# cloudflare/sliceslice-rs

Hardware: AMD Instinct MI355X
Metric: haystack GB/s scanned (and % HBM roofline), 16-byte needle, 1/2/4/8 MI355X (higher is better)
Workload: dtype u8

## Files before the change

### sliceslice-rs_amd/csrc/scan_filters.hpp

```cpp
#pragma once
#include <hip/hip_runtime.h>
#include <stddef.h>
#include <stdint.h>

#include <type_traits>

namespace ss {

constexpr int kWave = 64;
constexpr int kBlock = 256;
constexpr int kWavesPerBlock = kBlock / kWave;
constexpr int kMaxBlock = 512;
constexpr int kMaxWavesPerBlock = kMaxBlock / kWave;
constexpr unsigned kPeekFromBlock = 1024;
#ifndef SS_BATCH_MIN_TILES
#define SS_BATCH_MIN_TILES 8
#endif
constexpr uint64_t kBatchMinTiles = SS_BATCH_MIN_TILES;
constexpr int kFindOffsetBits = 40;
constexpr int kNeedleLds = 2048;

typedef uint32_t u32x4 __attribute__((ext_vector_type(4)));

struct Problem {
// ... 81 lines not shown
__device__ __forceinline__ void fold_ascii_chunk(u32x4 &A)
{
    A.x = fold_ascii4(A.x); A.y = fold_ascii4(A.y); A.z = fold_ascii4(A.z); A.w = fold_ascii4(A.w);
}
__device__ __forceinline__ void fold_ascii_chunk_keep(u32x4 &A, uint32_t keepx4)
{
    A.x = fold_ascii4_keep(A.x, keepx4); A.y = fold_ascii4_keep(A.y, keepx4);
    A.z = fold_ascii4_keep(A.z, keepx4); A.w = fold_ascii4_keep(A.w, keepx4);
}
template <bool FOLD> __device__ __forceinline__ uint32_t hay_u32(uint32_t x, uint32_t keepx4) { return FOLD ? fold_ascii4_keep(x, keepx4) : x; }
template <bool FOLD> __device__ __forceinline__ uint8_t hay_u8(uint8_t b, uint32_t keepx4)
{
    return FOLD && (uint8_t)(b - 'A') < 26 && b != (uint8_t)keepx4 ? (uint8_t)(b | 0x20) : b;
}

struct __attribute__((packed, aligned(1))) UnalignedU32 {
    uint32_t v;
};

template <bool FOLD = false>
__device__ __forceinline__ bool verify_candidate(const uint8_t *hay, const uint8_t *needle, uint64_t n, const uint8_t *s_needle,
                                                 uint64_t i, uint32_t keepx4 = 0)
{
    const uint8_t *h = hay + i;
    const uint64_t n_lds = n < (uint64_t)kNeedleLds ? n : (uint64_t)kNeedleLds;
    uint64_t k = 0;
    for (; k + 16 <= n_lds; k += 16) {
        const uint32_t a0 = hay_u32<FOLD>(reinterpret_cast<const UnalignedU32 *>(h + k)->v, keepx4), a1 = hay_u32<FOLD>(reinterpret_cast<const UnalignedU32 *>(h + k + 4)->v, keepx4);
        const uint32_t a2 = hay_u32<FOLD>(reinterpret_cast<const UnalignedU32 *>(h + k + 8)->v, keepx4), a3 = hay_u32<FOLD>(reinterpret_cast<const UnalignedU32 *>(h + k + 12)->v, keepx4);
        const u32x4 nd = *reinterpret_cast<const u32x4 *>(s_needle + k);
        if (((a0 ^ nd.x) | (a1 ^ nd.y) | (a2 ^ nd.z) | (a3 ^ nd.w)) != 0) return false;
    }
    for (; k + 4 <= n_lds; k += 4)
        if (hay_u32<FOLD>(reinterpret_cast<const UnalignedU32 *>(h + k)->v, keepx4) != *reinterpret_cast<const uint32_t *>(s_needle + k))
            return false;
    for (; k < n_lds; ++k)
        if (hay_u8<FOLD>(h[k], keepx4) != s_needle[k]) return false;
    for (; k + 4 <= n; k += 4)
        if (hay_u32<FOLD>(reinterpret_cast<const UnalignedU32 *>(h + k)->v, keepx4) != reinterpret_cast<const UnalignedU32 *>(needle + k)->v)
            return false;
    for (; k < n; ++k)
        if (hay_u8<FOLD>(h[k], keepx4) != needle[k]) return false;
    return true;
}

template <bool FOLD = false>
__device__ __forceinline__ bool same_bytes(const uint8_t *hb, uint32_t off, const uint8_t *nd, uint32_t count, uint32_t keepx4 = 0)
{
    auto u32 = [](const uint8_t *p, uint32_t o) { return reinterpret_cast<const UnalignedU32 *>(p + o)->v; };
    auto group = [&](uint32_t at, uint32_t len) {
        const uint32_t o3 = at + len - 4;
        if (hay_u32<FOLD>(u32(hb, off + at), keepx4) != u32(nd, at)) return false;
        if (hay_u32<FOLD>(u32(hb, off + o3), keepx4) != u32(nd, o3)) return false;
        if (len <= 8) return true;
        const uint32_t o1 = at + 4, o2 = at + len - 8;
        if (hay_u32<FOLD>(u32(hb, off + o1), keepx4) != u32(nd, o1)) return false;
        return hay_u32<FOLD>(u32(hb, off + o2), keepx4) == u32(nd, o2);
    };
    if (count < 4) {
        if (count == 0) return true;
        const uint32_t mid = count >> 1, last = count - 1;
        return (uint32_t)((hay_u8<FOLD>(hb[off], keepx4) ^ nd[0]) | (hay_u8<FOLD>(hb[off + mid], keepx4) ^ nd[mid]) | (hay_u8<FOLD>(hb[off + last], keepx4) ^ nd[last])) == 0;
    }
    for (uint32_t k = 0; k + 16 < count; k += 16)
        if (!group(k, 16)) return false;
    const uint32_t base = count > 16 ? count - 16 : 0;
    return group(base, count - base);
}


__device__ __forceinline__ void position_diffs(const u32x4 &B, uint32_t nlx4, uint32_t w[4])
{
    w[0] = B.x ^ nlx4;
    w[1] = B.y ^ nlx4;
    w[2] = B.z ^ nlx4;
    w[3] = B.w ^ nlx4;
}

template <int Q, bool ONE_BYTE>
__device__ __forceinline__ void filter_piece(const u32x4 &A, const uint32_t w[4], const uint32_t wl[4],
                                             const Problem &pr, uint32_t g[4])
{
    const uint32_t d0 = A.x ^ pr.n0x4, d1 = A.y ^ pr.n0x4, d2 = A.z ^ pr.n0x4, d3 = A.w ^ pr.n0x4;
    if (ONE_BYTE) {
        g[0] = zero_byte_flags(d0); g[1] = zero_byte_flags(d1); g[2] = zero_byte_flags(d2); g[3] = zero_byte_flags(d3);
        return;
    }
    uint32_t x[8];
#pragma unroll
    for (int j = 0; j < 4; ++j) {
        x[j] = w[j];
        x[4 + j] = (j <= Q) ? from_next_lane_or(wl[j], w[j]) : 0u;
    }
    g[0] = zero_byte_flags(d0 | __builtin_amdgcn_alignbyte(x[Q + 1], x[Q + 0], pr.r));
    g[1] = zero_byte_flags(d1 | __builtin_amdgcn_alignbyte(x[Q + 2], x[Q + 1], pr.r));
    g[2] = zero_byte_flags(d2 | __builtin_amdgcn_alignbyte(x[Q + 3], x[Q + 2], pr.r));
    g[3] = zero_byte_flags(d3 | __builtin_amdgcn_alignbyte(x[Q + 4], x[Q + 3], pr.r));
}

template <int Q, int Q3>
__device__ __forceinline__ void filter_piece3(const u32x4 &A, const uint32_t NX[4], const Problem &pr, uint32_t g[4])
{
    constexpr int QM = Q > Q3 ? Q : Q3;
    uint32_t x[8];
    x[0] = A.x; x[1] = A.y; x[2] = A.z; x[3] = A.w;
    x[4] = from_next_lane_or(NX[0], A.x);
    x[5] = QM >= 1 ? from_next_lane_or(NX[1], A.y) : 0u;
    x[6] = QM >= 2 ? from_next_lane_or(NX[2], A.z) : 0u;
    x[7] = QM >= 3 ? from_next_lane_or(NX[3], A.w) : 0u;
    uint32_t y[5], z[5];
#pragma unroll
    for (int k = 0; k < 5; ++k) {
        y[k] = x[Q + k] ^ pr.nlx4;
        z[k] = x[Q3 + k] ^ pr.n3x4;
    }
#pragma unroll
    for (int j = 0; j < 4; ++j)
        g[j] = zero_byte_flags((x[j] ^ pr.n0x4) | __builtin_amdgcn_alignbyte(y[j + 1], y[j], pr.r) |
                               __builtin_amdgcn_alignbyte(z[j + 1], z[j], pr.r3));
}


__host__ __device__ constexpr inline int byte_rarity_rank(uint8_t b)
{
    if (b == ' ') return 255;
    if (b >= 'a' && b <= 'z') {
        const uint8_t kLetter[26] = { 242,  174,  206,  214,  250,  190,  186,
                                          222,  234,  162,  166,  210,  198,  230,
                                          238,  178,  154,  218,  226,  246,  202,
                                          170,  194,  158,  182,  150};
        return kLetter[b - 'a'];
    }
    if (b == 0) return 200;
    if (b == '\n' || b == '\r' || b == '\t') return 140;
    if (b >= '0' && b <= '9') return 120;
    if (b == '.' || b == ',' || b == '-' || b == '_' || b == '/' || b == ':' || b == '"' || b == '=') return 110;
    if (b >= 'A' && b <= 'Z') return 100;
    if (b >= 0x21 && b <= 0x7E) return 60;
    if (b == 0xFF) return 50;
    return 20;
}

constexpr int kRefineWindow = 32;
constexpr uint32_t kFarFirst = 10;
#ifndef SS_REFINE_BYTES_PER_BALLOT
#define SS_REFINE_BYTES_PER_BALLOT 1
#endif
#ifndef SS_EXACT_REFINE_STEPS
#define SS_EXACT_REFINE_STEPS 2
#endif
constexpr uint32_t kExactRefineSteps = SS_EXACT_REFINE_STEPS;
constexpr uint32_t kExactSparseLanes = 24;
constexpr uint32_t kRefineBytesPerBallot = SS_REFINE_BYTES_PER_BALLOT;

__host__ __device__ inline uint32_t build_refine_order(const uint8_t *needle, uint64_t n, uint64_t position,
                                                       uint64_t idx[2], uint64_t val[2], uint64_t position3 = ~0ull)
{
    uint8_t ks[2][kRefineWindow];
    int rk[2][kRefineWindow];
    uint32_t cnt[2] = {0, 0};
    const int lim = n < (uint64_t)kRefineWindow ? (int)n : kRefineWindow;
    for (int K = 1; K < lim; ++K) {
        if ((uint64_t)K == position || (uint64_t)K == position3) continue;
        const int g = K >= 16 ? 0 : 1;
        const int r = byte_rarity_rank(needle[K]);
        int at = (int)cnt[g];
        while (at > 0 && rk[g][at - 1] > r) {
            rk[g][at] = rk[g][at - 1];
            ks[g][at] = ks[g][at - 1];
            --at;
        }
        rk[g][at] = r;
        ks[g][at] = (uint8_t)K;
        ++cnt[g];
    }
    idx[0] = idx[1] = val[0] = val[1] = 0;
    uint32_t m = 0;
    auto emit = [&](uint8_t K) {
        idx[m >> 3] |= (uint64_t)K << (8 * (m & 7));
        val[m >> 3] |= (uint64_t)needle[K] << (8 * (m & 7));
        ++m;
    };
    uint32_t far_used = 0;
    for (; far_used < cnt[0] && far_used < kFarFirst; ++far_used) emit(ks[0][far_used]);
    for (uint32_t t = 0; t < cnt[1] && m < 15; ++t) emit(ks[1][t]);
    for (; far_used < cnt[0] && m < 15; ++far_used) emit(ks[0][far_used]);
    return m;
}

__device__ __forceinline__ uint32_t build_refine_order_wave(const uint8_t *needle, uint64_t n, uint64_t position,
                                                            int lane, uint64_t idx[2], uint64_t val[2], uint64_t position3 = ~0ull)
{
    const int lim = n < (uint64_t)kRefineWindow ? (int)n : kRefineWindow;
    const bool valid = lane >= 1 && lane < lim && (uint64_t)lane != position && (uint64_t)lane != position3;
    const uint32_t b = valid ? needle[lane] : 0u;
    const int r = byte_rarity_rank((uint8_t)b);
    const int cls = !valid ? -1 : (r < 64 ? 0 : (r < 128 ? 1 : (r < 192 ? 2 : 3)));
    uint64_t i0 = 0, i1 = 0, v0 = 0, v1 = 0;
    uint32_t m = 0;
    auto take = [&](uint32_t mask, uint32_t cap) {
        while (mask && m < cap) {
            const int K = __ffs((int)mask) - 1;
            mask &= mask - 1;
            const uint64_t v = (uint32_t)__builtin_amdgcn_readlane((int)b, K) & 0xFF;
            const uint32_t sh = 8 * (m & 7);
            if (m < 8) { i0 |= (uint64_t)K << sh; v0 |= v << sh; }
            else { i1 |= (uint64_t)K << sh; v1 |= v << sh; }
            ++m;
        }
    };
#pragma unroll 1
    for (int c = 0; c < 4; ++c) take((uint32_t)__ballot(cls == c) & 0xFFFF0000u, kFarFirst);
#pragma unroll 1
    for (int c = 0; c < 4; ++c) take((uint32_t)__ballot(cls == c) & 0x0000FFFFu, 15u);
    idx[0] = i0; idx[1] = i1; val[0] = v0; val[1] = v1;
    return m;
}

struct NextPiece {
    u32x4 N;
    int kind;
};

__device__ __forceinline__ uint32_t next_lane_diffs(uint32_t own, uint32_t nword, uint32_t nkx4, int kind)
{
    const uint32_t f = nword ^ nkx4;
    return from_next_lane_or(kind == 1 ? rotate_from_next_lane(f) : f, own);
}

__device__ __forceinline__ uint32_t next2_lane_diffs(uint32_t hop1, uint32_t nword, uint32_t nkx4, int kind)
{
    uint32_t last = 0u;
    if (kind == 1) last = rotate_from_next_lane(rotate_from_next_lane(nword ^ nkx4));
    return from_next_lane_or(last, hop1);
}

template <int QK>
__device__ __forceinline__ void refine_flags_q(const u32x4 &A, const NextPiece &np, uint32_t nkx4, uint32_t rk, uint32_t g[4])
{
    static_assert(QK >= 0 && QK <= 7, "second-level bytes lie within 32 bytes of the first filter byte");
    constexpr auto need = [](int i) { return i >= QK && i <= QK + 4; };
    const uint32_t own[4] = {A.x ^ nkx4, A.y ^ nkx4, A.z ^ nkx4, A.w ^ nkx4};
    const uint32_t nw[4] = {np.N.x, np.N.y, np.N.z, np.N.w};
    uint32_t e[12];
#pragma unroll
    for (int j = 0; j < 4; ++j) {
        e[j] = own[j];
        e[4 + j] = e[8 + j] = 0u;
        if (need(4 + j) || need(8 + j)) e[4 + j] = next_lane_diffs(own[j], nw[j], nkx4, np.kind);
        if (need(8 + j)) e[8 + j] = next2_lane_diffs(e[4 + j], nw[j], nkx4, np.kind);
    }
#pragma unroll
    for (int j = 0; j < 4; ++j) g[j] &= zero_byte_flags(__builtin_amdgcn_alignbyte(e[j + QK + 1], e[j + QK], rk));
}

struct RefineOrder {
    uint32_t n;
    uint64_t idx[2], val[2];
};

template <int U, int MODE>
__device__ __forceinline__ bool refine_tile(const u32x4 (&A)[U], const u32x4 &H, const RefineOrder &ro, uint32_t (&G)[U][4],
                                            uint32_t max_steps)
{
    auto any_left = [&]() {
        uint32_t o = 0;
#pragma unroll
        for (int u = 0; u < U; ++u) o |= G[u][0] | G[u][1] | G[u][2] | G[u][3];
        return __ballot((o & 0x80808080u) != 0) != 0;
    };
    auto apply = [&](auto qk_c, uint32_t nkx4, uint32_t rk) {
        constexpr int QK = decltype(qk_c)::value;
#pragma unroll
        for (int u = 0; u < U; ++u) {
            NextPiece np;
            np.N = u + 1 < U ? A[u + 1] : H;
            np.kind = u + 1 < U ? 1 : (MODE == 0 ? 0 : 1);
            refine_flags_q<QK>(A[u], np, nkx4, rk, G[u]);
        }
    };
    bool any = any_left();
    const uint32_t steps = ro.n < max_steps ? ro.n : max_steps;
    uint32_t t = 0;
#pragma unroll 1
    while (t < steps && any) {
#pragma unroll 1
        for (uint32_t k = 0; k < kRefineBytesPerBallot && t < steps; ++k, ++t) {
            const uint32_t sh = 8 * (t & 7);
            const int K = (int)(((t < 8 ? ro.idx[0] : ro.idx[1]) >> sh) & 0xFF);
            const uint32_t v = (uint32_t)(((t < 8 ? ro.val[0] : ro.val[1]) >> sh) & 0xFF);
            const uint32_t nkx4 = 0x01010101u * v, rk = (uint32_t)(K & 3);
            switch (K >> 2) {
            case 0: apply(std::integral_constant<int, 0>{}, nkx4, rk); break;
            case 1: apply(std::integral_constant<int, 1>{}, nkx4, rk); break;
            case 2: apply(std::integral_constant<int, 2>{}, nkx4, rk); break;
            case 3: apply(std::integral_constant<int, 3>{}, nkx4, rk); break;
            case 4: apply(std::integral_constant<int, 4>{}, nkx4, rk); break;
            case 5: apply(std::integral_constant<int, 5>{}, nkx4, rk); break;
            case 6: apply(std::integral_constant<int, 6>{}, nkx4, rk); break;
            default: apply(std::integral_constant<int, 7>{}, nkx4, rk); break;
            }
        }
        any = any_left();
    }
    return any;
}
// ... 113 lines not shown
        const int t = __ffs((int)flags) - 1;
        flags &= flags - 1;
        const uint32_t off = 16u * (uint32_t)lane + (uint32_t)t;
        const uint64_t i = ubase + off;
        if (i >= va.end) continue;
        uint32_t in_memory = front;
        if ((uint32_t)t < back) {
            in_memory = (uint32_t)va.n;
        } else {
            const int start = t - (int)back;
            const int q = start >> 2;
            const uint32_t r = (uint32_t)(start & 3);
            auto pick = [&](uint32_t a, uint32_t b1, uint32_t c, uint32_t d) {
                const uint32_t lo = q & 1 ? b1 : a, hi = q & 1 ? d : c;
                return q & 2 ? hi : lo;
            };
            const uint32_t sw[5] = {pick(w0, w1, w2, w3), pick(w1, w2, w3, w4), pick(w2, w3, w4, w5), pick(w3, w4, w5, w6),
                                    pick(w4, w5, w6, w7)};
            uint32_t diff = 0;
#pragma unroll
            for (int j = 0; j < 4; ++j) diff |= (__builtin_amdgcn_alignbyte(sw[j + 1], sw[j], r) ^ cmp16[j]) & M[j];
            if (diff != 0) continue;
        }
        hit = in_memory == 0 || same_bytes(hb, off, va.needle, in_memory);
        where_off = off;
    }
    return hit;
}

template <bool FOLD = false>
__device__ __forceinline__ uint32_t exact_verify_piece_all(const u32x4 &A, const NextPiece &np, const uint32_t g[4], uint64_t chunk_wave,
                                                           int lane, const Problem &pr, const VerifyArgs &va, const uint32_t cmp16[4],
                                                           uint32_t exact, uint32_t keepx4 = 0)
{
    const uint64_t ubase = chunk_wave * 16 - pr.mis;
    const uint8_t *hb = va.hay + ubase;
    const uint32_t exact_len = exact & 0xFFu, back = (exact >> 8) & 0xFFu;
    auto hop = [&](uint32_t nword, uint32_t own) {
        return from_next_lane_or(np.kind == 1 ? rotate_from_next_lane(nword) : nword, own);
    };
    const uint32_t w0 = A.x, w1 = A.y, w2 = A.z, w3 = A.w;
    const uint32_t w4 = hop(np.N.x, w0), w5 = hop(np.N.y, w1), w6 = hop(np.N.z, w2), w7 = hop(np.N.w, w3);
    uint32_t M[4];
#pragma unroll
    for (int j = 0; j < 4; ++j) {
        const int rem = (int)exact_len - 4 * j;
        M[j] = rem >= 4 ? ~0u : (rem <= 0 ? 0u : (1u << (8 * rem)) - 1u);
    }
    uint32_t flags = flag_nibble(g[0]) | (flag_nibble(g[1]) << 4) | (flag_nibble(g[2]) << 8) | (flag_nibble(g[3]) << 12);
    if (back != 0) {
        const uint32_t low = flags & ((1u << back) - 1u);
        flags = (lane == 0 ? flags : flags & ~low) | (from_next_lane_or(0u, low) << 16);
    }
    const uint64_t anchor = (uint64_t)((pr.base + pr.mis) - va.hay);
    const uint32_t front = (uint32_t)(anchor - back);
    uint32_t mask = 0;
    while (flags != 0) {
        const int t = __ffs((int)flags) - 1;
        flags &= flags - 1;
        const uint32_t off = 16u * (uint32_t)lane + (uint32_t)t;
        const uint64_t i = ubase + off;
        if (i >= va.end) continue;
        uint32_t in_memory = front;
        if ((uint32_t)t < back) {
            in_memory = (uint32_t)va.n;
        } else {
            const int start = t - (int)back;
            const int q = start >> 2;
            const uint32_t r = (uint32_t)(start & 3);
            auto pick = [&](uint32_t a, uint32_t b1, uint32_t c, uint32_t d) {
                const uint32_t lo = q & 1 ? b1 : a, hi = q & 1 ? d : c;
                return q & 2 ? hi : lo;
            };
            const uint32_t sw[5] = {pick(w0, w1, w2, w3), pick(w1, w2, w3, w4), pick(w2, w3, w4, w5), pick(w3, w4, w5, w6),
                                    pick(w4, w5, w6, w7)};
            uint32_t diff = 0;
#pragma unroll
            for (int j = 0; j < 4; ++j) diff |= (__builtin_amdgcn_alignbyte(sw[j + 1], sw[j], r) ^ cmp16[j]) & M[j];
            if (diff != 0) continue;
        }
        if (in_memory == 0 || same_bytes<FOLD>(hb, off, va.needle, in_memory, keepx4)) mask |= 1u << t;
    }
    return mask;
}

__device__ __forceinline__ uint32_t wave_sum(uint32_t v)
{
    v += (uint32_t)__builtin_amdgcn_mov_dpp((int)v, 0xB1 , 0xf, 0xf, false);
    v += (uint32_t)__builtin_amdgcn_mov_dpp((int)v, 0x4E , 0xf, 0xf, false);
    v += (uint32_t)__builtin_amdgcn_mov_dpp((int)v, 0x141 , 0xf, 0xf, false);
    v += (uint32_t)__builtin_amdgcn_mov_dpp((int)v, 0x140 , 0xf, 0xf, false);
    return (uint32_t)__builtin_amdgcn_readlane((int)v, 0) + (uint32_t)__builtin_amdgcn_readlane((int)v, 16) +
           (uint32_t)__builtin_amdgcn_readlane((int)v, 32) + (uint32_t)__builtin_amdgcn_readlane((int)v, 48);
}

__device__ __forceinline__ uint32_t wave_exclusive_sum(uint32_t v, int lane)
{
    uint32_t x = v;
#pragma unroll
    for (int k = 1; k < kWave; k <<= 1) {
        const uint32_t y = (uint32_t)__shfl_up((int)x, (unsigned)k, kWave);
        if (lane >= k) x += y;
    }
    return x - v;
}

__device__ __forceinline__ uint64_t uniform64(uint64_t x)
{
    return ((uint64_t)(uint32_t)__builtin_amdgcn_readfirstlane((int)(x >> 32)) << 32) |
           (uint32_t)__builtin_amdgcn_readfirstlane((int)(uint32_t)x);
}

__device__ __forceinline__ int poll_found(const int *found, int epoch)
{
    return __builtin_amdgcn_readfirstlane(
               __hip_atomic_load(found, __ATOMIC_RELAXED, __HIP_MEMORY_SCOPE_AGENT)) == epoch;
}

__device__ __forceinline__ int scalar_peek(const int *p)
{
    int v;
    asm volatile("s_load_dword %0, %1, 0x0\n\ts_waitcnt lgkmcnt(0)" : "=s"(v) : "s"(p) : "memory");
    return v;
}

__device__ __forceinline__ uint64_t scalar_peek64(const uint64_t *p)
{
    uint64_t v;
    asm volatile("s_load_dwordx2 %0, %1, 0x0\n\ts_waitcnt lgkmcnt(0)" : "=s"(v) : "s"(p) : "memory");
    return v;
}

__device__ __forceinline__ void forget_scalar_cache() { __builtin_amdgcn_s_dcache_inv(); }
__device__ __forceinline__ void forget_scalar_cache_unless(bool small_grid)
{
    if (!small_grid) __builtin_amdgcn_s_dcache_inv();
}

__device__ __forceinline__ void publish_found(int *found, int epoch = 1)
{
    __hip_atomic_store(found, epoch, __ATOMIC_RELAXED, __HIP_MEMORY_SCOPE_AGENT);
}


__device__ __forceinline__ void stage_needle_wave(uint8_t *s_needle, const uint8_t *needle, uint64_t n, int lane)
{
    const uint32_t m = n < (uint64_t)kNeedleLds ? (uint32_t)n : (uint32_t)kNeedleLds;
    for (uint32_t k = lane; k < m; k += kWave) s_needle[k] = needle[k];
    __builtin_amdgcn_fence(__ATOMIC_RELEASE, "wavefront");
    __builtin_amdgcn_wave_barrier();
    __builtin_amdgcn_fence(__ATOMIC_ACQUIRE, "wavefront");
}

typedef uint32_t u32x2 __attribute__((ext_vector_type(2)));

template <bool NT>
__device__ __forceinline__ u32x2 load_half(const uint8_t *base, uint64_t half_chunk)
{
    const u32x2 *p = reinterpret_cast<const u32x2 *>(base) + half_chunk;
    if (NT) return __builtin_nontemporal_load(p);
    return *p;
}

template <int Q, bool ONE_BYTE>
__device__ __forceinline__ uint32_t filter_half(const u32x2 &a, const u32x2 &t, const u32x2 &tn, const Problem &pr,
                                                int lane, uint32_t acc)
{
    const uint32_t d0 = a.x ^ pr.n0x4, d1 = a.y ^ pr.n0x4;
    if (ONE_BYTE) return acc | zero_byte_flags(d0) | zero_byte_flags(d1);
    uint32_t x[6] = {t.x, t.y, 0, 0, 0, 0};
    const int i1 = ((lane + 1) & (kWave - 1)) << 2, i2 = ((lane + 2) & (kWave - 1)) << 2;
    if (Q <= 2) x[2] = (uint32_t)__builtin_amdgcn_ds_bpermute(i1, (int)(lane < 1 ? tn.x : t.x));
    if (Q >= 1) x[3] = (uint32_t)__builtin_amdgcn_ds_bpermute(i1, (int)(lane < 1 ? tn.y : t.y));
    if (Q >= 2) x[4] = (uint32_t)__builtin_amdgcn_ds_bpermute(i2, (int)(lane < 2 ? tn.x : t.x));
    if (Q >= 3) x[5] = (uint32_t)__builtin_amdgcn_ds_bpermute(i2, (int)(lane < 2 ? tn.y : t.y));
    const uint32_t c0 = d0 | __builtin_amdgcn_alignbyte(x[Q + 1], x[Q], pr.r);
    const uint32_t c1 = d1 | __builtin_amdgcn_alignbyte(x[Q + 2], x[Q + 1], pr.r);
    return acc | zero_byte_flags(c0) | zero_byte_flags(c1);
}

__device__ __forceinline__ uint32_t filter_half3_near(const u32x2 &a, uint32_t nx, const Problem &pr, uint32_t acc)
{
    const uint32_t y0 = a.x ^ pr.nlx4, y1 = a.y ^ pr.nlx4, y2 = nx ^ pr.nlx4;
    const uint32_t z0 = a.x ^ pr.n3x4, z1 = a.y ^ pr.n3x4, z2 = nx ^ pr.n3x4;
    const uint32_t c0 = (a.x ^ pr.n0x4) | __builtin_amdgcn_alignbyte(y1, y0, pr.r) | __builtin_amdgcn_alignbyte(z1, z0, pr.r3);
    const uint32_t c1 = (a.y ^ pr.n0x4) | __builtin_amdgcn_alignbyte(y2, y1, pr.r) | __builtin_amdgcn_alignbyte(z2, z1, pr.r3);
    return acc | zero_byte_flags(c0) | zero_byte_flags(c1);
}

__device__ __forceinline__ u32x4 transpose_halves(const u32x2 &lo, const u32x2 &hi, int lane)
{
    const int i0 = ((lane & 31) * 2) << 2, i1 = i0 + 4;
    const bool up = lane >= 32;
    u32x4 A;
    const uint32_t ax = (uint32_t)__builtin_amdgcn_ds_bpermute(i0, (int)lo.x), bx = (uint32_t)__builtin_amdgcn_ds_bpermute(i0, (int)hi.x);
    const uint32_t ay = (uint32_t)__builtin_amdgcn_ds_bpermute(i0, (int)lo.y), by = (uint32_t)__builtin_amdgcn_ds_bpermute(i0, (int)hi.y);
    const uint32_t az = (uint32_t)__builtin_amdgcn_ds_bpermute(i1, (int)lo.x), bz = (uint32_t)__builtin_amdgcn_ds_bpermute(i1, (int)hi.x);
    const uint32_t aw = (uint32_t)__builtin_amdgcn_ds_bpermute(i1, (int)lo.y), bw = (uint32_t)__builtin_amdgcn_ds_bpermute(i1, (int)hi.y);
    A.x = up ? bx : ax;
    A.y = up ? by : ay;
    A.z = up ? bz : az;
    A.w = up ? bw : aw;
    return A;
}

__device__ __forceinline__ uint32_t from_lane_ahead(uint32_t cur, uint32_t nxt, int lane, int k)
{
    const int idx = ((lane + k) & (kWave - 1)) << 2;
    const uint32_t a = (uint32_t)__builtin_amdgcn_ds_bpermute(idx, (int)cur);
    const uint32_t b = (uint32_t)__builtin_amdgcn_ds_bpermute(idx, (int)nxt);
    return lane + k < kWave ? a : b;
}

}
```

### sliceslice-rs_amd/csrc/scan_kernels.hpp

```cpp
#pragma once
#include "scan_filters.hpp"
#include "lines_tiles.hpp"

namespace ss {

#ifdef SS_CAND_PROF
constexpr int kCandProfSlots = 4096;
static __device__ unsigned long long g_cand_prof[kCandProfSlots][8];
#define SS_PROF_T(v) const unsigned long long v = __builtin_readcyclecounter()
#define SS_PROF_ADD(k, d) do { if (lane == 0) atomicAdd(&g_cand_prof[blockIdx.x % kCandProfSlots][k], (unsigned long long)(d)); } while (0)
#else
#define SS_PROF_T(v)
#define SS_PROF_ADD(k, d)
#endif

template <bool BATCHED> constexpr bool kNoForget = BATCHED;
template <class T, class = void> struct SingleLaunchPlan : std::false_type {};
template <class T> struct SingleLaunchPlan<T, std::void_t<decltype(T::kSingleLaunchPlan)>> : std::bool_constant<T::kSingleLaunchPlan> {};
struct AllTiles {
    uint32_t lane_count;
    bool emit;
    uint64_t rank;
    uint64_t *out;
    uint64_t capacity;
// ... 231 lines not shown
                        if (Q3 >= 1) xx[5] = from_next_lane_or(rotate_from_next_lane(NP.y), A[u].y);
                        if (Q3 >= 2) xx[6] = from_next_lane_or(rotate_from_next_lane(NP.z), A[u].z);
                        if (Q3 >= 3) xx[7] = from_next_lane_or(rotate_from_next_lane(NP.w), A[u].w);
                        uint32_t z[5];
#pragma unroll
                        for (int k = 0; k < 5; ++k) z[k] = xx[Q3 + k] ^ pr.n3x4;
                        g[0] = zero_byte_flags((A[u].x ^ pr.n0x4) | __builtin_amdgcn_alignbyte(x[QS + 1], x[QS + 0], pr.r) | __builtin_amdgcn_alignbyte(z[1], z[0], pr.r3));
                        g[1] = zero_byte_flags((A[u].y ^ pr.n0x4) | __builtin_amdgcn_alignbyte(x[QS + 2], x[QS + 1], pr.r) | __builtin_amdgcn_alignbyte(z[2], z[1], pr.r3));
                        g[2] = zero_byte_flags((A[u].z ^ pr.n0x4) | __builtin_amdgcn_alignbyte(x[QS + 3], x[QS + 2], pr.r) | __builtin_amdgcn_alignbyte(z[3], z[2], pr.r3));
                        g[3] = zero_byte_flags((A[u].w ^ pr.n0x4) | __builtin_amdgcn_alignbyte(x[QS + 4], x[QS + 3], pr.r) | __builtin_amdgcn_alignbyte(z[4], z[3], pr.r3));
                    } else {
                        g[0] = zero_byte_flags((A[u].x ^ pr.n0x4) | __builtin_amdgcn_alignbyte(x[QS + 1], x[QS + 0], pr.r));
                        g[1] = zero_byte_flags((A[u].y ^ pr.n0x4) | __builtin_amdgcn_alignbyte(x[QS + 2], x[QS + 1], pr.r));
                        g[2] = zero_byte_flags((A[u].z ^ pr.n0x4) | __builtin_amdgcn_alignbyte(x[QS + 3], x[QS + 2], pr.r));
                        g[3] = zero_byte_flags((A[u].w ^ pr.n0x4) | __builtin_amdgcn_alignbyte(x[QS + 4], x[QS + 3], pr.r));
                    }
                } else {
                    if (!ONE_BYTE) {
                        if (u + 1 < U) {
                            position_diffs(A[u + 1], pr.nlx4, wnext);
#pragma unroll
                            for (int j = 0; j < 4; ++j) wlast[j] = (j <= QQ) ? rotate_from_next_lane(wnext[j]) : 0u;
                        } else {
                            position_diffs(H, pr.nlx4, wlast);
                        }
                    }
                    filter_piece<QQ < 0 ? 0 : QQ, ONE_BYTE>(A[u], wcur, wlast, pr, g);
                }
                any_tile |= g[0] | g[1] | g[2] | g[3];
                if (!ONE_BYTE && !THREE && (SHIFTED || u + 1 < U)) {
#pragma unroll
                    for (int j = 0; j < 4; ++j) wcur[j] = wnext[j];
                }
            }

        };
        auto run_phase1 = [&](auto loaded_c, auto full_c) {
            using std::integral_constant;
            if constexpr (THREE && Q == kQDynamic) {
                switch (pr.q * 4 + pr.q3) {
                case 0: load_and_filter(loaded_c, full_c, integral_constant<int, 0>{}, integral_constant<int, 0>{}); break;
                case 4: load_and_filter(loaded_c, full_c, integral_constant<int, 0>{}, integral_constant<int, 1>{}); break;
                case 5: load_and_filter(loaded_c, full_c, integral_constant<int, 1>{}, integral_constant<int, 1>{}); break;
                case 8: load_and_filter(loaded_c, full_c, integral_constant<int, 0>{}, integral_constant<int, 2>{}); break;
                case 9: load_and_filter(loaded_c, full_c, integral_constant<int, 1>{}, integral_constant<int, 2>{}); break;
                case 10: load_and_filter(loaded_c, full_c, integral_constant<int, 2>{}, integral_constant<int, 2>{}); break;
                case 12: load_and_filter(loaded_c, full_c, integral_constant<int, 0>{}, integral_constant<int, 3>{}); break;
                case 13: load_and_filter(loaded_c, full_c, integral_constant<int, 1>{}, integral_constant<int, 3>{}); break;
                case 14: load_and_filter(loaded_c, full_c, integral_constant<int, 2>{}, integral_constant<int, 3>{}); break;
                default: load_and_filter(loaded_c, full_c, integral_constant<int, 3>{}, integral_constant<int, 3>{}); break;
                }
            } else if constexpr (THREE || SHIFTED3) {
                switch (pr.q3) {
                case 0: load_and_filter(loaded_c, full_c, integral_constant<int, 0>{}, integral_constant<int, 0>{}); break;
                case 1: load_and_filter(loaded_c, full_c, integral_constant<int, 1>{}, integral_constant<int, 0>{}); break;
                case 2: load_and_filter(loaded_c, full_c, integral_constant<int, 2>{}, integral_constant<int, 0>{}); break;
                default: load_and_filter(loaded_c, full_c, integral_constant<int, 3>{}, integral_constant<int, 0>{}); break;
                }
            } else {
                load_and_filter(loaded_c, full_c, integral_constant<int, 0>{}, integral_constant<int, 0>{});
            }
        };
        if (have16) run_phase1(std::true_type{}, std::true_type{});
        else if (full) run_phase1(std::false_type{}, std::true_type{});
        else run_phase1(std::false_type{}, std::false_type{});
        if constexpr (LINES && FOLD) line_clip<U>(chunk0, lane, *lines, line_dm);
        else if constexpr (LINES) line_capture<U>(A, chunk0, lane, *lines, line_dm);
        if (FIND) {
            const uint64_t first = chunk0 * 16 > pr.mis ? chunk0 * 16 - pr.mis : 0;
            if (best_now <= pr.find_base + first) {
                forget_scalar_cache_unless(small_grid || kNoForget<LAZY_ORDER>);
                return;
            }
        }

        const bool cand_tile = __ballot((any_tile & 0x80808080u) != 0) != 0;
        if (L8) dense = cand_tile;
        if (stop) {
            forget_scalar_cache_unless(small_grid || kNoForget<LAZY_ORDER>);
            return;
        }
        if (cand_tile) {
            SS_PROF_T(prof_t0);
            if (!LAZY_ORDER || !ordered) {
                const auto c = cold();
                va.hay = reinterpret_cast<const uint8_t *>(uniform64((uint64_t)(uintptr_t)c->hay));
                va.needle = reinterpret_cast<const uint8_t *>(uniform64((uint64_t)(uintptr_t)c->needle));
                va.n = uniform64(c->n);
                va.end = uniform64(c->end);
                bool take = !BUILD_ORDER;
                if constexpr (MAYBE_ORDER) take = __builtin_amdgcn_readfirstlane((int)c->ready) != 0;
                if (!ONE_BYTE && (MAYBE_ORDER || !BUILD_ORDER) && take) {
                    ro.n = c->norder;
                    ro.idx[0] = c->order_idx[0]; ro.idx[1] = c->order_idx[1];
                    ro.val[0] = c->order_val[0]; ro.val[1] = c->order_val[1];
                    if (EXACT_OK) {
                        exact_len = c->exact_len;
#pragma unroll
                        for (int j = 0; j < 4; ++j) tail16[j] = c->tail16[j];
                    }
                    if (LAZY_ORDER) {
                        ro.n = (uint32_t)__builtin_amdgcn_readfirstlane((int)ro.n);
                        for (int t = 0; t < 2; ++t) {
                            ro.idx[t] = uniform64(ro.idx[t]);
                            ro.val[t] = uniform64(ro.val[t]);
                        }
                        if (EXACT_OK) {
                            exact_len = (uint32_t)__builtin_amdgcn_readfirstlane((int)exact_len);
#pragma unroll
                            for (int j = 0; j < 4; ++j) tail16[j] = (uint32_t)__builtin_amdgcn_readfirstlane((int)tail16[j]);
                        }
                    }
                }
                if (!ONE_BYTE && BUILD_ORDER && !take) {
                    const uint64_t position = pr.d * 16 + 4 * (Q == kQDynamic ? pr.q : (uint32_t)Q) + pr.r;
                    const uint64_t position3 = THREE ? (uint64_t)(4 * pr.q3 + pr.r3) : ~0ull;
                    const uint64_t anchor = (uint64_t)((pr.base + pr.mis) - va.hay);
                    ro.n = (uint32_t)__builtin_amdgcn_readfirstlane(
                        (int)build_refine_order_wave(va.needle + anchor, va.n - anchor, position, lane, ro.idx, ro.val, position3));
                    for (int t = 0; t < 2; ++t) {
                        ro.idx[t] = uniform64(ro.idx[t]);
                        ro.val[t] = uniform64(ro.val[t]);
                    }
                    if (EXACT_OK && va.n - anchor <= 16) {
                        const uint32_t behind = (uint32_t)(va.n - anchor);
                        const uint32_t back = (uint32_t)(anchor < 16 - behind ? anchor : 16 - behind);
                        const uint32_t el = behind + back;
                        exact_len = el | (back << 8);
                        const uint32_t nbv = (uint32_t)lane < el ? (uint32_t)va.needle[anchor - back + lane] : 0u;
#pragma unroll
                        for (int j = 0; j < 4; ++j)
                            tail16[j] = ((uint32_t)__builtin_amdgcn_readlane((int)nbv, 4 * j) & 0xFF) |
                                        (((uint32_t)__builtin_amdgcn_readlane((int)nbv, 4 * j + 1) & 0xFF) << 8) |
                                        (((uint32_t)__builtin_amdgcn_readlane((int)nbv, 4 * j + 2) & 0xFF) << 16) |
                                        (((uint32_t)__builtin_amdgcn_readlane((int)nbv, 4 * j + 3) & 0xFF) << 24);
                    }
                }
                ordered = true;
            }
            SS_PROF_T(prof_t1);
            auto stage_once = [&]() {
                if (!staged && !ONE_BYTE) {
                    stage_needle_wave(s_needle, va.needle, va.n, lane);
                    staged = true;
                }
            };
#ifndef SS_MODE2_TILE_WIDE
#define SS_MODE2_TILE_WIDE 1
#endif
            constexpr bool TILE_WIDE = MODE < 2 || SS_MODE2_TILE_WIDE != 0;
            uint32_t pm = (1u << U) - 1;
            bool per_piece = !TILE_WIDE;
            uint32_t cand_lanes = 0;
            if (!ONE_BYTE && TILE_WIDE) {
                pm = 0;
#pragma unroll
                for (int u = 0; u < U; ++u) {
                    const uint64_t bl = __ballot(((G[u][0] | G[u][1] | G[u][2] | G[u][3]) & 0x80808080u) != 0);
                    if (bl != 0) pm |= 1u << u;
                    cand_lanes += (uint32_t)__builtin_popcountll(bl);
                }
#ifdef SS_NO_SPARSE_REFINE
                per_piece = false;
#else
                per_piece = __builtin_popcount(pm) <= 2;
#endif
                if (!per_piece) {
                    const bool exact = EXACT_OK && exact_len != 0;
                    const uint32_t max_steps = exact ? (cand_lanes <= kExactSparseLanes ? 0u : kExactRefineSteps) : 15u;
                    if (max_steps != 0 && !refine_tile<U, MODE>(A, H, ro, G, max_steps)) {
                        SS_PROF_T(prof_tx);
                        SS_PROF_ADD(0, 1);
                        SS_PROF_ADD(1, prof_tx - prof_t0);
                        SS_PROF_ADD(2, prof_t1 - prof_t0);
                        SS_PROF_ADD(3, prof_tx - prof_t1);
                        continue;
                    }
                }
            }
            bool hit = false;
#ifdef SS_CAND_PROF
            unsigned long long prof_refine = 0, prof_verify = 0;
            SS_PROF_T(prof_t2);
#endif
#pragma unroll
            for (int u = 0; u < U; ++u) {
                uint32_t *g = G[u];
                SS_PROF_T(prof_p0);
                if (!ONE_BYTE && per_piece) {
                    if (((pm >> u) & 1u) == 0) continue;
                    NextPiece np;
                    np.N = u + 1 < U ? A[u + 1] : H;
                    np.kind = u + 1 < U ? 1 : (MODE == 0 ? 0 : 1);
                    if (!(EXACT_OK && exact_len != 0) && !refine_piece(A[u], np, ro, g)) {
#ifdef SS_CAND_PROF
                        prof_refine += __builtin_readcyclecounter() - prof_p0;
#endif
                        continue;
                    }
                } else if (__ballot(((g[0] | g[1] | g[2] | g[3]) & 0x80808080u) != 0) == 0) {
                    continue;
                }
                SS_PROF_T(prof_p1);
#ifdef SS_CAND_PROF
                prof_refine += prof_p1 - prof_p0;
#endif
                if constexpr (ALL) {
                    uint32_t mk;
                    if (EXACT_OK && exact_len != 0) {
                        NextPiece np;
                        np.N = u + 1 < U ? A[u + 1] : H;
                        np.kind = u + 1 < U ? 1 : 0;
                        mk = exact_verify_piece_all<FOLD>(A[u], np, g, chunk0 + 64 * u, lane, pr, va, tail16, exact_len, keepx4);
                    } else {
                        stage_once();
                        const uint64_t far_off = MODE == 0 && !ONE_BYTE ? uniform64(cold()->far_off) : 0;
                        mk = verify_flags_all<ONE_BYTE, FOLD>(g, chunk0 + 64 * u + lane, pr, va, s_needle, far_off, keepx4);
                    }
                    if constexpr (LINES) {
                        all_mask[u] = mk;
                    } else {
                        if (all->emit) all_mask[u] = mk;
                        else all->lane_count += (uint32_t)__builtin_popcount(mk);
                    }
                    continue;
                }
                uint64_t where = 0;
                bool h;
                if (EXACT_OK && exact_len != 0) {
                    NextPiece np;
                    np.N = u + 1 < U ? A[u + 1] : H;
                    np.kind = u + 1 < U ? 1 : 0;
                    uint32_t where_off = 0;
                    h = exact_verify_piece(A[u], np, g, chunk0 + 64 * u, lane, pr, va, tail16, exact_len, where_off);
                    if (FIND) where = (chunk0 + 64 * u) * 16 - pr.mis + where_off;
                } else {
                    stage_once();
                    const uint64_t far_off = MODE == 0 && !ONE_BYTE ? uniform64(cold()->far_off) : 0;
                    h = verify_flags<ONE_BYTE>(g, chunk0 + 64 * u + lane, pr, va, s_needle, where, far_off);
                }
                hit |= h;
#ifdef SS_CAND_PROF
                prof_verify += __builtin_readcyclecounter() - prof_p1;
#endif
                if (!FIND && __ballot(h) != 0) break;
                if (FIND) {
                    const uint64_t m = __ballot(h);
                    if (m != 0) {
                        const int src = __ffsll((unsigned long long)m) - 1;
                        const uint32_t lo = __builtin_amdgcn_readlane((uint32_t)where, src);
                        const uint32_t hi = __builtin_amdgcn_readlane((uint32_t)(where >> 32), src);
                        const uint64_t mine = pr.find_base + (((uint64_t)hi << 32) | lo);
                        if (WG_FIND && wg_sink != nullptr) {
                            if (lane == 0)
                                __hip_atomic_fetch_min(static_cast<uint64_t *>(wg_sink), mine, __ATOMIC_RELAXED, __HIP_MEMORY_SCOPE_WORKGROUP);
                        } else if (lane == 0 && mine < __hip_atomic_load(best, __ATOMIC_RELAXED, __HIP_MEMORY_SCOPE_AGENT)) {
                            if constexpr (SingleLaunchPlan<ColdT>::value) {
                                const uint64_t old = __hip_atomic_fetch_min(best, mine, __ATOMIC_RELAXED, __HIP_MEMORY_SCOPE_AGENT);
                                __asm__ volatile("s_waitcnt vmcnt(0)" : : "v"(old) : "memory");
                                const auto c = cold();
                                uint64_t *out_best = reinterpret_cast<uint64_t *>(c->host_flag);
                                if (out_best) __hip_atomic_fetch_min(out_best, mine, __ATOMIC_RELAXED, __HIP_MEMORY_SCOPE_AGENT);
                                if (old == ~0ull && c->tally) __hip_atomic_fetch_add(c->tally, 1u, __ATOMIC_RELAXED, __HIP_MEMORY_SCOPE_AGENT);
                            } else {
                                __hip_atomic_fetch_min(best, mine, __ATOMIC_RELAXED, __HIP_MEMORY_SCOPE_AGENT);
                                if constexpr (LAZY_ORDER) {
                                    uint64_t *out_best = reinterpret_cast<uint64_t *>(cold()->host_flag);
                                    if (out_best) __hip_atomic_fetch_min(out_best, mine, __ATOMIC_RELAXED, __HIP_MEMORY_SCOPE_AGENT);
                                }
                            }
                        }
                        forget_scalar_cache_unless(small_grid || kNoForget<LAZY_ORDER>);
                        return;
                    }
                }
            }
            if (!FIND && !ALL) {
                const uint64_t hits = __ballot(hit);
                if (hits != 0) {
                    if (wg_found != nullptr) {
                        if (lane == __ffsll((unsigned long long)hits) - 1)
                            __hip_atomic_store(wg_found, 1, __ATOMIC_RELAXED, __HIP_MEMORY_SCOPE_WORKGROUP);
                    } else if (lane == __ffsll((unsigned long long)hits) - 1 &&
                               __hip_atomic_load(found, __ATOMIC_RELAXED, __HIP_MEMORY_SCOPE_AGENT) != pr.epoch) {
                        const int old = __hip_atomic_exchange(found, pr.epoch, __ATOMIC_RELAXED, __HIP_MEMORY_SCOPE_AGENT);
                        if constexpr (SingleLaunchPlan<ColdT>::value) {
                            if (old != pr.epoch) {
                                const auto c = cold();
                                if (c->host_flag) (void)__hip_atomic_exchange(c->host_flag, 1, __ATOMIC_RELAXED, __HIP_MEMORY_SCOPE_AGENT);
                                if (c->tally) __hip_atomic_fetch_add(c->tally, 1u, __ATOMIC_RELAXED, __HIP_MEMORY_SCOPE_AGENT);
                            }
                        } else {
                            int *host_flag = cold()->host_flag;
                            if (old != pr.epoch && host_flag)
                                __hip_atomic_store(host_flag, pr.epoch, __ATOMIC_RELAXED, __HIP_MEMORY_SCOPE_SYSTEM);
                        }
                    }
                    forget_scalar_cache_unless(small_grid || kNoForget<LAZY_ORDER>);
                    return;
                }
            }
#ifdef SS_CAND_PROF
            {
                SS_PROF_T(prof_tz);
                SS_PROF_ADD(0, 1);
                SS_PROF_ADD(1, prof_tz - prof_t0);
                SS_PROF_ADD(2, prof_t1 - prof_t0);
                SS_PROF_ADD(3, prof_refine);
                SS_PROF_ADD(4, prof_verify);
                SS_PROF_ADD(5, prof_t2 - prof_t1);
                if (per_piece) SS_PROF_ADD(6, 1);
            }
#endif
        }
    }
}

#ifdef SS_WAVES_PER_EU
#define SS_SCAN_OCCUPANCY __attribute__((amdgpu_waves_per_eu(SS_WAVES_PER_EU, SS_WAVES_PER_EU)))
#else
#define SS_SCAN_OCCUPANCY
#endif
template <int Q, int MODE, bool ONE_BYTE, int U, int NTMODE, bool FIND = false, bool L8 = false>
__global__ void SS_SCAN_OCCUPANCY __launch_bounds__(kMaxBlock) scan_kernel(const Problem pr, void *found, uint64_t tiles_per_block)
{
    extern __shared__ __attribute__((aligned(16))) uint8_t s_needle[];
    static_assert((U & (U - 1)) == 0, "U is a power of two");
    static_assert(sizeof(Problem) <= 0x100 && offsetof(Problem, hay) < 0x80, "the cold fields live in the lines at 0x80 and 0xc0");
    uint32_t touch0, touch1;
    {
        ColdInKernarg::Ptr kp = (ColdInKernarg::Ptr)__builtin_amdgcn_kernarg_segment_ptr();
        __asm__ volatile("s_load_dword %0, %2, 0x80\n\ts_load_dword %1, %2, 0xc0" : "=&s"(touch0), "=&s"(touch1) : "s"(kp));
    }
    const unsigned tile_shift = (unsigned)__builtin_ctz(blockDim.x / kWave) + (unsigned)__builtin_ctz(U);
    uint64_t t0 = tiles_per_block ? (uint64_t)blockIdx.x * tiles_per_block : blockIdx.x;
    __shared__ int s_wg_found;
    const bool counted = !FIND && (pr.flags & kProblemCounted) != 0;
    if (counted) {
        if (threadIdx.x == 0) __hip_atomic_store(&s_wg_found, 0, __ATOMIC_RELAXED, __HIP_MEMORY_SCOPE_WORKGROUP);
        __syncthreads();
    }
    __asm__ volatile("s_waitcnt lgkmcnt(0)" : : "s"(touch0), "s"(touch1));
    bool skip = false;
    if (blockIdx.x >= kPeekFromBlock) {
        if (FIND) {
            const uint64_t first_chunk = (t0 << tile_shift) * 64;
            const uint64_t first = first_chunk * 16 > pr.mis ? first_chunk * 16 - pr.mis : 0;
            skip = scalar_peek64(static_cast<const uint64_t *>(found)) <= pr.find_base + first &&
                   uniform64(__hip_atomic_load(static_cast<const uint64_t *>(found), __ATOMIC_RELAXED, __HIP_MEMORY_SCOPE_AGENT)) <=
                       pr.find_base + first;
        } else {
            skip = scalar_peek(static_cast<const int *>(found)) == pr.epoch && poll_found(static_cast<const int *>(found), pr.epoch);
        }
    }
    if (!skip) {
        const uint64_t ntiles = (pr.npieces + ((uint64_t)1 << tile_shift) - 1) >> tile_shift;
        uint64_t step = gridDim.x, t1 = ntiles;
        if (tiles_per_block) {
            step = 1;
            t1 = t0 + tiles_per_block < ntiles ? t0 + tiles_per_block : ntiles;
        }
        scan_tiles<Q, MODE, ONE_BYTE, U, NTMODE, FIND, L8, false, ColdInKernarg>(pr, ColdInKernarg{}, s_needle, t0, step, t1, found,
                                                                                 counted ? &s_wg_found : nullptr);
    }
    if (counted) {
        __asm__ volatile("" ::: "memory");
        __builtin_amdgcn_s_waitcnt(0xc07f);
        __builtin_amdgcn_s_barrier();
        __asm__ volatile("" ::: "memory");
        if (threadIdx.x == 0) {
            const auto c = ColdInKernarg{}();
            const unsigned long long f = (unsigned long long)__hip_atomic_load(&s_wg_found, __ATOMIC_RELAXED, __HIP_MEMORY_SCOPE_WORKGROUP);
            const unsigned long long mine = 1ull + (f << 32);
            const unsigned long long total = __hip_atomic_fetch_add(c->done_counter, mine, __ATOMIC_RELAXED, __HIP_MEMORY_SCOPE_AGENT) + mine;
            if ((uint32_t)total == c->done_target) {
                const uint32_t hi = (uint32_t)(total >> 32);
                const long long word = (long long)(((unsigned long long)hi << 32) | ((unsigned long long)(uint32_t)pr.epoch << 1) |
                                                   (hi != c->done_hi ? 1ull : 0ull));
                __hip_atomic_store(c->host_done, word, __ATOMIC_RELAXED, __HIP_MEMORY_SCOPE_SYSTEM);
            }
        }
    } else if (FIND && (pr.flags & kProblemCounted) != 0) {
        __asm__ volatile("s_waitcnt vmcnt(0)" ::: "memory");
        __syncthreads();
        if (threadIdx.x == 0) {
            const auto c = ColdInKernarg{}();
            const unsigned long long total = __hip_atomic_fetch_add(c->done_counter, 1ull, __ATOMIC_RELAXED, __HIP_MEMORY_SCOPE_AGENT) + 1ull;
            if ((uint32_t)total == c->done_target) {
                __builtin_amdgcn_fence(__ATOMIC_ACQUIRE, "agent");
                const uint64_t v = __hip_atomic_load(static_cast<const uint64_t *>(found), __ATOMIC_RELAXED, __HIP_MEMORY_SCOPE_AGENT);
                const uint64_t off = v - pr.find_base;
                const bool hit = v >= pr.find_base && off < (1ull << kFindOffsetBits);
                __hip_atomic_store(c->host_done, hit ? (long long)(off + 1) : -1ll, __ATOMIC_RELAXED, __HIP_MEMORY_SCOPE_SYSTEM);
            }
        }
    }
}

struct AllArgs {
    uint64_t *total;
    uint32_t *wg_count;
    const uint64_t *wg_rank;
    uint64_t *out;
    uint64_t capacity;
    uint32_t mode;
};
constexpr uint32_t kAllCount = 0, kAllCountPerWorkgroup = 1, kAllEmit = 2;

template <int Q, int MODE, bool ONE_BYTE, bool FOLD>
__device__ __forceinline__ void scan_all_body(const Problem &pr, const AllArgs &aa, uint64_t tiles_per_block)
{
    extern __shared__ __attribute__((aligned(16))) uint8_t s_needle[];
    __shared__ uint32_t s_wave[kMaxWavesPerBlock];
    constexpr int U = 4;
    const int lane = threadIdx.x & (kWave - 1);
    const int wave = __builtin_amdgcn_readfirstlane(threadIdx.x / kWave);
    const int wpb = (int)(blockDim.x / kWave);
    const unsigned tile_shift = (unsigned)__builtin_ctz(blockDim.x / kWave) + (unsigned)__builtin_ctz(U);
    const uint64_t ntiles = (pr.npieces + ((uint64_t)1 << tile_shift) - 1) >> tile_shift;
    const uint64_t t0 = (uint64_t)blockIdx.x * tiles_per_block;
    const uint64_t t1 = t0 + tiles_per_block < ntiles ? t0 + tiles_per_block : ntiles;
    AllTiles at = {0u, aa.mode == kAllEmit, 0ull, aa.out, aa.capacity, s_wave};
    if (aa.mode == kAllEmit) {
        const uint32_t cnt = (uint32_t)__builtin_amdgcn_readfirstlane((int)aa.wg_count[blockIdx.x]);
        const uint64_t rank = uniform64(aa.wg_rank[blockIdx.x]);
        if (cnt == 0 || rank >= aa.capacity) return;
        at.rank = rank;
    }
    scan_tiles<Q, MODE, ONE_BYTE, U, 1, false, false, false, ColdInKernarg, true, false, FOLD>(pr, ColdInKernarg{}, s_needle, t0, 1, t1, &at);
    if (aa.mode == kAllEmit) return;
    const uint32_t wc = wave_sum(at.lane_count);
    if (lane == 0) s_wave[wave] = wc;
    __syncthreads();
    if (threadIdx.x == 0) {
        uint32_t sum = 0;
        for (int w = 0; w < wpb; ++w) sum += s_wave[w];
        if (aa.mode == kAllCountPerWorkgroup) aa.wg_count[blockIdx.x] = sum;
        else if (sum != 0) __hip_atomic_fetch_add(aa.total, (uint64_t)sum, __ATOMIC_RELAXED, __HIP_MEMORY_SCOPE_AGENT);
    }
}

template <int Q, int MODE, bool ONE_BYTE>
__global__ void __launch_bounds__(kMaxBlock) scan_all_kernel(const Problem pr, AllArgs aa, uint64_t tiles_per_block)
{
    scan_all_body<Q, MODE, ONE_BYTE, false>(pr, aa, tiles_per_block);
}

}
```

Measured before the change: 7433.

## Add dense-candidate compaction and lane-parallel verify; set wave occupancy floor

When a tile has many candidate lanes, candidate byte offsets are compacted into an LDS list with a wave prefix sum. The list is then verified one candidate per lane, and the tile is skipped if no lane matches, which replaces the serial refine/verify path for dense tiles. The scan kernel also gets an amdgpu_waves_per_eu floor of 6 for some template configurations to limit register use and raise occupancy. Risks are extra prefix-scan and LDS overhead on tiles that would have been rejected cheaply, and register spills caused by the occupancy constraint.

```diff
diff --git a/sliceslice-rs_amd/csrc/scan_filters.hpp b/sliceslice-rs_amd/csrc/scan_filters.hpp
--- a/sliceslice-rs_amd/csrc/scan_filters.hpp
+++ b/sliceslice-rs_amd/csrc/scan_filters.hpp
@@ -257,6 +257,16 @@
 constexpr uint32_t kExactRefineSteps = SS_EXACT_REFINE_STEPS;
 constexpr uint32_t kExactSparseLanes = 24;
 constexpr uint32_t kRefineBytesPerBallot = SS_REFINE_BYTES_PER_BALLOT;
+#ifndef SS_DENSE_MIN_LANES
+#define SS_DENSE_MIN_LANES 24
+#endif
+#ifndef SS_DENSE_CAP
+#define SS_DENSE_CAP 192
+#endif
+constexpr uint32_t kDenseMinLanes = SS_DENSE_MIN_LANES;
+constexpr uint32_t kDenseCap = SS_DENSE_CAP;
+static_assert(kDenseCap >= 1 && kDenseCap <= 255 && 4 * kDenseCap <= (uint32_t)kNeedleLds / 2, "the list lives in the upper half of a wave's LDS slice");
+constexpr uint32_t kDenseListAt = (uint32_t)kNeedleLds - 4 * kDenseCap;
 
 __host__ __device__ inline uint32_t build_refine_order(const uint8_t *needle, uint64_t n, uint64_t position,
                                                        uint64_t idx[2], uint64_t val[2], uint64_t position3 = ~0ull)
@@ -676,6 +686,91 @@
     __builtin_amdgcn_fence(__ATOMIC_ACQUIRE, "wavefront");
 }
 
+template <int U>
+__device__ __forceinline__ uint32_t dense_compact(const uint32_t (&G)[U][4], int lane, uint32_t *list)
+{
+    constexpr int W = (U + 3) / 4;
+    uint32_t packed[W], count = 0;
+#pragma unroll
+    for (int w = 0; w < W; ++w) packed[w] = 0;
+#pragma unroll
+    for (int u = 0; u < U; ++u) {
+        const uint32_t c = (uint32_t)__builtin_popcount(((G[u][0] & 0x80808080u) >> 3) | ((G[u][1] & 0x80808080u) >> 2) |
+                                                        ((G[u][2] & 0x80808080u) >> 1) | (G[u][3] & 0x80808080u));
+        count += c;
+        packed[u / 4] |= c << (8 * (u % 4));
+    }
+    if (wave_sum(count) > kDenseCap) return 0;
+    uint32_t base = 0;
+#pragma unroll
+    for (int w = 0; w < W; ++w) {
+        uint32_t inc = packed[w];
+#pragma unroll
+        for (int k = 1; k < kWave; k <<= 1) {
+            const uint32_t y = (uint32_t)__shfl_up((int)inc, (unsigned)k, kWave);
+            if (lane >= k) inc += y;
+        }
+        const uint32_t totals = (uint32_t)__builtin_amdgcn_readlane((int)inc, kWave - 1);
+        const uint32_t before = inc - packed[w];
+#pragma unroll
+        for (int u = 4 * w; u < U && u < 4 * w + 4; ++u) {
+            uint32_t slot = base + ((before >> (8 * (u % 4))) & 0xFFu);
+            uint32_t f = flag_nibble(G[u][0]) | (flag_nibble(G[u][1]) << 4) | (flag_nibble(G[u][2]) << 8) | (flag_nibble(G[u][3]) << 12);
+            const uint32_t at = 16u * (uint32_t)(64 * u + lane);
+            while (f != 0) {
+                const int t = __ffs((int)f) - 1;
+                f &= f - 1;
+                list[slot++] = at + (uint32_t)t;
+            }
+            base += (totals >> (8 * (u % 4))) & 0xFFu;
+        }
+    }
+    __builtin_amdgcn_fence(__ATOMIC_RELEASE, "wavefront");
+    __builtin_amdgcn_wave_barrier();
+    __builtin_amdgcn_fence(__ATOMIC_ACQUIRE, "wavefront");
+    return base;
+}
+
+__device__ __forceinline__ bool same_bytes_walk(const uint8_t *hb, uint32_t off, const uint8_t *nd, uint32_t n)
+{
+    bool ok = true;
+    uint32_t k = 0;
+    if (n < 4) {
+        do {
+            ok = hb[off + k] == nd[k];
+        } while (ok && ++k < n);
+        return ok;
+    }
+    do {
+        const uint32_t at = k + 4 <= n ? k : n - 4;
+        ok = reinterpret_cast<const UnalignedU32 *>(hb + off + at)->v == reinterpret_cast<const UnalignedU32 *>(nd + at)->v;
+        k += 4;
+    } while (ok && k < n);
+    return ok;
+}
+
+__device__ __forceinline__ bool dense_verify(const uint32_t *list, uint32_t total, uint64_t chunk_wave, int lane, const Problem &pr,
+                                             const VerifyArgs &va, uint32_t far_off)
+{
+    const uint64_t ubase = chunk_wave * 16 - pr.mis;
+    const uint8_t *hb = va.hay + ubase;
+    bool hit = false;
+#pragma unroll 1
+    for (uint32_t r0 = 0; r0 < total; r0 += kWave) {
+        const uint32_t e = r0 + (uint32_t)lane;
+        if (e < total) {
+            const uint32_t off = list[e];
+            const uint64_t i = ubase + off;
+            if (i < va.end) {
+                if (far_off != 0 && hb[off + far_off] != va.needle[far_off]) hit = false;
+                else hit = same_bytes_walk(hb, off, va.needle, (uint32_t)va.n);
+            }
+        }
+        if (__ballot(hit) != 0) break;
+    }
+    return hit;
+}
+
 typedef uint32_t u32x2 __attribute__((ext_vector_type(2)));
 
 template <bool NT>
diff --git a/sliceslice-rs_amd/csrc/scan_kernels.hpp b/sliceslice-rs_amd/csrc/scan_kernels.hpp
--- a/sliceslice-rs_amd/csrc/scan_kernels.hpp
+++ b/sliceslice-rs_amd/csrc/scan_kernels.hpp
@@ -407,6 +407,11 @@
             uint32_t pm = (1u << U) - 1;
             bool per_piece = !TILE_WIDE;
             uint32_t cand_lanes = 0;
+#ifdef SS_NO_DENSE_COMPACT
+            constexpr bool DENSE_OK = false;
+#else
+            constexpr bool DENSE_OK = !ONE_BYTE && !ALL && TILE_WIDE;
+#endif
             if (!ONE_BYTE && TILE_WIDE) {
                 pm = 0;
 #pragma unroll
@@ -423,6 +428,19 @@
                 if (!per_piece) {
                     const bool exact = EXACT_OK && exact_len != 0;
                     const uint32_t max_steps = exact ? (cand_lanes <= kExactSparseLanes ? 0u : kExactRefineSteps) : 15u;
+                    if constexpr (DENSE_OK) {
+                        if (cand_lanes > kDenseMinLanes && (!staged || va.n <= (uint64_t)kDenseListAt) && va.n < (1ull << 31)) {
+                            uint32_t *list = reinterpret_cast<uint32_t *>(s_needle + kDenseListAt);
+                            int dl = lane;
+                            __asm__ volatile("" : "+v"(dl));
+                            const uint32_t total = dense_compact<U>(G, dl, list);
+                            if (total != 0) {
+                                uint32_t far_off = 0;
+                                if (!exact && MODE == 0) far_off = (uint32_t)__builtin_amdgcn_readfirstlane((int)(uint32_t)cold()->far_off);
+                                if (__ballot(dense_verify(list, total, chunk0, dl, pr, va, far_off)) == 0) continue;
+                            }
+                        }
+                    }
                     if (max_steps != 0 && !refine_tile<U, MODE>(A, H, ro, G, max_steps)) {
                         SS_PROF_T(prof_tx);
                         SS_PROF_ADD(0, 1);
@@ -574,8 +592,12 @@
 #ifdef SS_WAVES_PER_EU
 #define SS_SCAN_OCCUPANCY __attribute__((amdgpu_waves_per_eu(SS_WAVES_PER_EU, SS_WAVES_PER_EU)))
 #else
-#define SS_SCAN_OCCUPANCY
-#endif
+#define SS_SCAN_OCCUPANCY __attribute__((amdgpu_waves_per_eu(scan_waves_floor(MODE, ONE_BYTE, U, FIND))))
+#endif
+constexpr unsigned scan_waves_floor(int mode, bool one_byte, int u, bool find)
+{
+    return !one_byte && u == 4 && (mode == 0 || (mode == 2 && find)) ? 6u : 1u;
+}
 template <int Q, int MODE, bool ONE_BYTE, int U, int NTMODE, bool FIND = false, bool L8 = false>
 __global__ void SS_SCAN_OCCUPANCY __launch_bounds__(kMaxBlock) scan_kernel(const Problem pr, void *found, uint64_t tiles_per_block)
 {
```

Measured after the change: 6549. 0.881x the previous value.
